# Xinjie-Q/Boosting-NeRV

Hardware: AMD Instinct MI355X
Metric: train frames/sec (higher is better)
Workload: dtype fp32; 1 GPU; NeRV-boost 1.5M (1489577 params, fc_dim 30) train step on a synthetic Bunny-shaped clip 132x3x720x1280: decoder fwd + Fusion10_freq + bwd + fused Adan; frames resident in HBM; global_batch=1, per_gpu_batch=1, parallelism=dp1, hipgraph=True, rccl_ranks=0, collective_in_graph=False

## Files before the change

boosting_nerv_amd/_lib.py:

```python
import ctypes as C
import os

import torch

_HERE = os.path.dirname(os.path.abspath(__file__))
LIB_PATH = os.environ.get("BNERV_LIB") or os.path.join(_HERE, "libbnerv_hip.so")

MAX_DENSE_GROUPS = 40
ADAN_MAX_TENSORS = 48
SFT_CHUNKS = 32
LOSS_STATS = 5
DENSE_DX_CHUNK = 64

ACT_NONE, ACT_RELU, ACT_SIN = 0, 1, 2
IN_PLAIN, IN_AFFINE, IN_GELU_AFFINE, IN_UNSHUFFLE, IN_TANHGRAD = 0, 1, 2, 3, 4
EP_BIAS, EP_BIAS_SIN, EP_BIAS_RES, EP_BIAS_TANH, EP_PLAIN, EP_DGELU, EP_DSIN, EP_BIAS_GELU, EP_DGELU_SAVED = 0, 1, 2, 3, 4, 5, 6, 7, 8
CONV_FAM = ("head1_fwd", "head1_dgrad", "head3", "stem_dgrad", "small", "small96", "wide_bf16", "q4", "generic")
WGRAD_FAM = ("stem", "gemm1x1", "lean", "wide_bf16", "wide_f32", "generic")
PAIR_FORM = ("stem", "q4_lean", "small_wide", "bf16_wide", "head")

_fp = C.c_void_p


class DenseFwdDesc(C.Structure):
# ... 2 lines not shown


class DenseBwdDesc(C.Structure):
    _fields_ = [("x", _fp), ("w", _fp), ("y", _fp), ("aux", _fp), ("dy", _fp), ("dpre", _fp), ("dw", _fp), ("db", _fp),
                ("dx_part", _fp), ("I", C.c_int), ("O", C.c_int), ("act", C.c_int), ("_pad", C.c_int)]


class ConvDesc(C.Structure):
    _fields_ = [("x", _fp), ("w", _fp), ("bias", _fp), ("out", _fp), ("out2", _fp), ("aux0", _fp), ("aux1", _fp),
                ("aux2", _fp), ("scale", _fp), ("shift", _fp), ("partial", _fp),
                ("B", C.c_int), ("Cin", C.c_int), ("Cout", C.c_int), ("H", C.c_int), ("W", C.c_int), ("k", C.c_int),
                ("in_mode", C.c_int), ("ep_mode", C.c_int), ("in_s", C.c_int), ("out_s", C.c_int),
                ("transposed", C.c_int), ("wCo", C.c_int), ("wCi", C.c_int), ("ctx", _fp)]


class TimeBranchMlp(C.Structure):
    _fields_ = [("w1", _fp), ("b1", _fp), ("w2", _fp), ("b2", _fp), ("hs", _fp), ("out", _fp), ("C", C.c_int), ("_pad", C.c_int)]


class TimeBranchDesc(C.Structure):
    _fields_ = [("pos", _fp), ("bases", _fp), ("pe", _fp), ("sw0", _fp), ("sb0", _fp), ("sy0", _fp), ("saux0", _fp),
                ("tw0", _fp), ("tb0", _fp), ("tw1", _fp), ("tb1", _fp), ("ty0", _fp), ("taux0", _fp), ("ty1", _fp), ("taux1", _fp),
                ("B", C.c_int), ("L", C.c_int), ("SH", C.c_int), ("TH", C.c_int), ("TO", C.c_int), ("n_mlp", C.c_int)]


class WgradDesc(C.Structure):
    _fields_ = [("x", _fp), ("g", _fp), ("gaux", _fp), ("scale", _fp), ("shift", _fp), ("dw", _fp), ("db", _fp),
                ("ws", _fp), ("ws_bytes", C.c_size_t),
                ("B", C.c_int), ("Cin", C.c_int), ("Cout", C.c_int), ("H", C.c_int), ("W", C.c_int), ("k", C.c_int),
                ("in_mode", C.c_int), ("g_mode", C.c_int), ("g_s", C.c_int), ("defer_finish", C.c_int), ("ctx", _fp)]


class LossDesc(C.Structure):
    _fields_ = [("pred", _fp), ("target", _fp), ("grad", _fp), ("loss_out", _fp), ("stats_out", _fp), ("ws", _fp),
                ("ws_bytes", C.c_size_t), ("B", C.c_int), ("C", C.c_int), ("H", C.c_int), ("W", C.c_int),
                ("c_l1", C.c_float), ("c_l2", C.c_float), ("c_ms", C.c_float), ("c_fft", C.c_float)]


class AdanChunk(C.Structure):
    _fields_ = [("p", _fp * ADAN_MAX_TENSORS), ("g", _fp * ADAN_MAX_TENSORS), ("exp_avg", _fp * ADAN_MAX_TENSORS),
                ("exp_avg_sq", _fp * ADAN_MAX_TENSORS), ("exp_avg_diff", _fp * ADAN_MAX_TENSORS),
                ("neg_pre_grad", _fp * ADAN_MAX_TENSORS), ("n", C.c_int * ADAN_MAX_TENSORS), ("n_tensors", C.c_int)]


class AdanHyper(C.Structure):
    _fields_ = [("beta1", C.c_float), ("beta2", C.c_float), ("beta3", C.c_float), ("eps", C.c_float),
# ... 106 lines not shown


PRUNE_SLICE = 16384


class PruneItem(C.Structure):
    _fields_ = [("x", _fp), ("mask", _fp), ("n", C.c_uint32), ("_pad", C.c_uint32)]


class YuvCoeffs(C.Structure):
    _fields_ = [("m", C.c_float * 9), ("off", C.c_float * 3), ("scale", C.c_float * 3), ("maxcode", C.c_float)]


_I, _Z, _V, _F = C.c_int, C.c_size_t, C.c_void_p, C.c_float
SYMBOLS = {
    "bnerv_abi_version": (_I, []),
    "bnerv_last_error": (C.c_char_p, []),
    "bnerv_build_arch": (C.c_char_p, []),
    "bnerv_pe_fwd_f32": (_I, [_V, _V, _V, _V, _I, _I]),
    "bnerv_pe_fwd_f64": (_I, [_V, _V, _V, _V, _I, _I]),
    "bnerv_pe_fwd_f32_from_f64": (_I, [_V, _V, _V, _V, _I, _I]),
    "bnerv_dense_grouped_fwd": (_I, [_V, C.POINTER(DenseFwdDesc), _I, _I]),
    "bnerv_time_branch_fwd": (_I, [_V, C.POINTER(TimeBranchDesc), C.POINTER(TimeBranchMlp)]),
    "bnerv_dense_grouped_bwd": (_I, [_V, C.POINTER(DenseBwdDesc), _I, _I]),
    "bnerv_sft_affine_fwd": (_I, [_V, _V, _V, _V, _V, _I, _I, _I]),
    "bnerv_sft_affine_bwd": (_I, [_V, _V, _V, _V, _V, _V, _I, _I, _I]),
    "bnerv_reduce_slabs": (_I, [_V, _V, _I, _I, _V]),
    "bnerv_ctx_create": (_I, [C.POINTER(C.c_void_p)]),
    "bnerv_ctx_destroy": (None, [_V]),
    "bnerv_ctx_scratch_bytes": (_Z, [_V]),
    "bnerv_ctx_reserve": (_I, [_V, _Z]),
    "bnerv_ctx_wplan_record": (_I, [_V]),
    "bnerv_ctx_wplan_freeze": (_I, [_V]),
    "bnerv_ctx_wplan_run": (_I, [_V, _V]),
    "bnerv_ctx_wplan_run_fetch": (_I, [_V, _V, _V, _V, _V, _I, _Z, _V, _V]),
    "bnerv_ctx_wplan_end": (_I, [_V]),
    "bnerv_ctx_wplan_entries": (_I, [_V]),
    "bnerv_reduce_slabs_deferred": (_I, [_V, _V, _V, _I, _I, _V]),
    "bnerv_flush_deferred": (_I, [_V, _V]),
    "bnerv_deferred_pending": (_I, [_V]),
    "bnerv_conv_tiles": (_I, [_I, _I]),
    "bnerv_conv_igemm": (_I, [_V, C.POINTER(ConvDesc)]),
    "bnerv_conv_splitk_ws_bytes": (_Z, [C.POINTER(ConvDesc)]),
    "bnerv_conv_partial_rows": (_I, [C.POINTER(ConvDesc)]),
    "bnerv_conv_family": (_I, [C.POINTER(ConvDesc), C.POINTER(C.c_int)]),
    "bnerv_conv_wgrad_ws_bytes": (_Z, [_I, _I, _I, _I, _I, _I]),
# ... 243 lines not shown
```

boosting_nerv_amd/csrc/abi.hip:

```cpp
#include "common.h"
#include <string.h>

namespace { thread_local char g_err[512] = ""; }

int bnerv_set_error(int code, const char* fmt, ...) {
    va_list ap;
    va_start(ap, fmt);
    vsnprintf(g_err, sizeof(g_err), fmt, ap);
    va_end(ap);
    return code;
}

extern "C" int bnerv_abi_version(void) { return BNERV_ABI_VERSION; }
extern "C" const char* bnerv_last_error(void) { return g_err; }
extern "C" const char* bnerv_build_arch(void) { return "gfx950"; }

#include "sidejob.h"
#include <new>
#include <vector>

namespace {
__global__ __launch_bounds__(256) void side_flush_kernel(const SidePack sp) {
    __shared__ float red[256];
    side_slice<SidePack, true>(sp, blockIdx.x, red);
}
__global__ __launch_bounds__(256) void side_flush_many_kernel(const SideFlushPack sp) {
    __shared__ float red[256];
    side_slice<SideFlushPack, true>(sp, blockIdx.x, red);
}

SideJob make_job(const void* src, int n_slabs, int count, int ncols, float* out, float* out2, const float* fs = nullptr, const float* ft = nullptr) {
    SideJob j;
    j.fs = fs;
    j.ft = ft;
    j.src = reinterpret_cast<const float*>(src);
    j.out = out;
    j.out2 = out2;
    j.n_slabs = n_slabs;
    j.count = count;
    j.ncols = ncols;
    int lanes = 8;
    while (lanes < 128 && lanes * 16 < n_slabs) lanes *= 2;
    j.epb = 256 / lanes;
    j.slices = (count + j.epb - 1) / j.epb;
    return j;
}
}

void bnerv_side_push(bnerv_ctx* ctx, hipStream_t st, const void* src, int n_slabs, int count, int ncols, float* out, float* out2, const float* fold_scale, const float* fold_shift) {
    const SideJob j = make_job(src, n_slabs, count, ncols, out, out2, fold_scale, fold_shift);
    if (ctx) { ctx->queue.push_back(j); return; }
    SidePack sp;
    sp.j[0] = j;
    sp.n_jobs = 1;
    sp.n_slices = j.slices;
    hipLaunchKernelGGL(side_flush_kernel, dim3(sp.n_slices), dim3(256), 0, st, sp);
}

void bnerv_side_take(bnerv_ctx* ctx, SidePack* sp, int max_slices, bool step_over) {
    sp->n_jobs = 0;
    sp->n_slices = 0;
    if (!ctx) return;
    std::vector<SideJob>& q = ctx->queue;
    int n = 0;
    size_t i = 0;
    while (i < q.size() && n < SIDE_MAX_JOBS) {
// ... 86 lines not shown
```

boosting_nerv_amd/csrc/dense.hip:

```cpp
#include "common.h"
#include "sidejob.h"
#include "launch.h"

namespace {

__global__ void pe_f32_kernel(const float* __restrict__ pos, const float* __restrict__ bases, float* __restrict__ out, int N, int L) {
    const int i = blockIdx.x * blockDim.x + threadIdx.x;
    if (i >= N * L) return;
    const int n = i / L, l = i - n * L;
    const float v = __fmul_rn(pos[n], bases[l]);
    out[(size_t)n * 2 * L + l] = sinf(v);
    out[(size_t)n * 2 * L + L + l] = cosf(v);
}
__global__ void pe_f32_from_f64_kernel(const double* __restrict__ pos, const float* __restrict__ bases, float* __restrict__ out, int N, int L) {
    const int i = blockIdx.x * blockDim.x + threadIdx.x;
    if (i >= N * L) return;
    const int n = i / L, l = i - n * L;
    const float v = __fmul_rn((float)pos[n], bases[l]);
    out[(size_t)n * 2 * L + l] = sinf(v);
    out[(size_t)n * 2 * L + L + l] = cosf(v);
}
__global__ void pe_f64_kernel(const double* __restrict__ pos, const float* __restrict__ bases, float* __restrict__ out, int N, int L) {
    const int i = blockIdx.x * blockDim.x + threadIdx.x;
    if (i >= N * L) return;
// ... 16 lines not shown
    for (int b = 0; b < ap->B; ++b) {
        const float* x = g.x + (size_t)b * g.I;
        float s = 0.f;
        for (int i = lane; i < g.I; i += 64) s = fmaf(wrow[i], x[i], s);
        s = wave_sum(s);
        if (lane == 0) {
            const float pre = s + bias;
            float y = pre;
            if (g.act == BNERV_ACT_RELU) y = fmaxf(pre, 0.f);
            else if (g.act == BNERV_ACT_SIN) {
                float sv, cv;
                sincosf(pre, &sv, &cv);
                y = sv;
                if (g.aux) g.aux[(size_t)b * g.O + o] = cv;
            }
            g.y[(size_t)b * g.O + o] = y;
        }
    }
}

struct BwdArgs { bnerv_dense_bwd_desc g[BNERV_MAX_DENSE_GROUPS]; int B; };

constexpr int DW_CHUNK = 1024;
__device__ __forceinline__ void dense_bwd_w_body(const BwdArgs& a, const int bx, const int by, const int bz) {
    const BwdArgs* ap = &a;
    const bnerv_dense_bwd_desc g = a.g[by];
    const int lane = threadIdx.x & 63, wave = threadIdx.x >> 6;
    const int o = bx * 4 + wave;
    const int i0 = bz * DW_CHUNK;
    if (o >= g.O || (i0 >= g.I && bz != 0)) return;
    const int B = ap->B;
    if (bz == 0) {
        float dbsum = 0.f;
        for (int b = 0; b < B; ++b) {
            const size_t k = (size_t)b * g.O + o;
            float dp = g.dy[k];
            if (g.act == BNERV_ACT_RELU) dp = g.y[k] > 0.f ? dp : 0.f;
            else if (g.act == BNERV_ACT_SIN) dp *= g.aux[k];
            if (lane == 0) g.dpre[k] = dp;
            dbsum += dp;
        }
        if (lane == 0 && g.db) g.db[o] = dbsum;
    }
    const int i1 = min(i0 + DW_CHUNK, g.I);
    for (int ib = i0 + lane; ib < i1; ib += 256) {
        float s[4] = {0.f, 0.f, 0.f, 0.f};
        for (int b = 0; b < B; ++b) {
            const size_t k = (size_t)b * g.O + o;
            float dp = g.dy[k];
            if (g.act == BNERV_ACT_RELU) dp = g.y[k] > 0.f ? dp : 0.f;
            else if (g.act == BNERV_ACT_SIN) dp *= g.aux[k];
#pragma unroll
            for (int u = 0; u < 4; ++u) {
                const int i = ib + 64 * u;
                if (i < i1) s[u] = fmaf(dp, g.x[(size_t)b * g.I + i], s[u]);
            }
        }
#pragma unroll
        for (int u = 0; u < 4; ++u) {
            const int i = ib + 64 * u;
            if (i < i1) g.dw[(size_t)o * g.I + i] = s[u];
        }
    }
}

__device__ __forceinline__ void dense_bwd_x_body(const BwdArgs& a, const int bx, const int by, const int bz) {
    const BwdArgs* ap = &a;
    const bnerv_dense_bwd_desc g = a.g[bz];
    if (!g.dx_part) return;
    const int chunk = bx;
    const int o0 = chunk * BNERV_DENSE_DX_CHUNK;
    if (o0 >= g.O) return;
    const int o1 = min(o0 + BNERV_DENSE_DX_CHUNK, g.O);
    const int b = by;
    __shared__ float s_dp[BNERV_DENSE_DX_CHUNK];
    if ((int)threadIdx.x < BNERV_DENSE_DX_CHUNK) {
        float dp = 0.f;
        if ((int)threadIdx.x < o1 - o0) {
            const size_t k = (size_t)b * g.O + o0 + threadIdx.x;
            dp = g.dy[k];
            if (g.act == BNERV_ACT_RELU) dp = g.y[k] > 0.f ? dp : 0.f;
            else if (g.act == BNERV_ACT_SIN) dp *= g.aux[k];
        }
        s_dp[threadIdx.x] = dp;
    }
    __syncthreads();
    for (int i = threadIdx.x; i < g.I; i += 256) {
        float wv[BNERV_DENSE_DX_CHUNK];
#pragma unroll
        for (int r = 0; r < BNERV_DENSE_DX_CHUNK; ++r) wv[r] = o0 + r < o1 ? g.w[(size_t)(o0 + r) * g.I + i] : 0.f;
        float s = 0.f;
#pragma unroll
        for (int r = 0; r < BNERV_DENSE_DX_CHUNK; ++r) s = fmaf(s_dp[r], wv[r], s);
        g.dx_part[((size_t)chunk * ap->B + b) * g.I + i] = s;
    }
}

struct BwdGrid { int nw, wpre[BNERV_MAX_DENSE_GROUPS + 1], xpre[BNERV_MAX_DENSE_GROUPS + 1]; int n_groups, B; };
__global__ __launch_bounds__(256) void dense_bwd_kernel(const BwdArgs a, const BwdGrid q) {
    int t = blockIdx.x;
    const int* pre = t < q.nw ? q.wpre : q.xpre;
    const bool wphase = t < q.nw;
    if (!wphase) t -= q.nw;
    const int ln = threadIdx.x & 63;
    const bool ge = ln + 1 < q.n_groups && t >= pre[ln + 1];
// ... 226 lines not shown
        s_t0[b][r] = sv;
        if (cb == 0) { d.ty0[(size_t)b * d.TH + r] = sv; d.taux0[(size_t)b * d.TH + r] = cv; }
    }
    __syncthreads();
    tb_rows16<TB_MAXT>(w_t1, b_t1, d.TH, TO, s_t0, &s_zt[0][0], TB_MAXT, B);
    __syncthreads();
    for (int e = tid; e < B * TO; e += TB_NT) {
        const int b = e / TO, r = e - b * TO;
        float sv, cv;
        sincosf(s_zt[b][r], &sv, &cv);
        s_zt[b][r] = sv;
        if (cb == 0) { d.ty1[(size_t)b * TO + r] = sv; d.taux1[(size_t)b * TO + r] = cv; }
    }
    __syncthreads();
    tb_multi8(nm, TO, TO, B, [&](int) { return TO; }, [&](int k) { return w_m + k * mstride; }, [&](int k) { return b_m + k * bstride; },
              [&](int, int b) { return &s_zt[b][0]; },
              [&](int k, int r, int b, float v) { const float y = fmaxf(v, 0.f); s_h[k][b][r] = y; a.m[m0 + k].hs[(size_t)b * TO + r] = y; });
    __syncthreads();
    tb_multi8(nm, a.cmax, TO, B, [&](int k) { return a.m[m0 + k].C; }, [&](int k) { return w_m + k * mstride + TO * TO; }, [&](int k) { return b_m + k * bstride + TB_MAXO; },
              [&](int k, int b) { return &s_h[k][b][0]; },
              [&](int k, int r, int b, float v) { a.m[m0 + k].out[(size_t)b * a.m[m0 + k].C + r] = v; });
}

extern "C" int bnerv_dense_grouped_fwd(void* stream, const bnerv_dense_fwd_desc* groups, int n_groups, int B) {
    BNERV_REQUIRE(groups && n_groups > 0 && n_groups <= BNERV_MAX_DENSE_GROUPS && B > 0, "dense_grouped_fwd: bad args (n_groups=%d)", n_groups);
    FwdArgs a;
    a.B = B;
    int maxO = 0;
    for (int i = 0; i < n_groups; ++i) {
        BNERV_REQUIRE(groups[i].x && groups[i].w && groups[i].y && groups[i].I > 0 && groups[i].O > 0, "dense_grouped_fwd: bad group %d", i);
        a.g[i] = groups[i];
        if (groups[i].O > maxO) maxO = groups[i].O;
    }
    hipStream_t st = (hipStream_t)stream;
    hipLaunchKernelGGL(dense_fwd_kernel, dim3(cdiv(maxO, 4), n_groups), dim3(256), 0, st, a);
    BNERV_LAUNCH_CHECK("dense_fwd");
    return BNERV_OK;
}

extern "C" int bnerv_dense_grouped_bwd(void* stream, const bnerv_dense_bwd_desc* groups, int n_groups, int B) {
    BNERV_REQUIRE(groups && n_groups > 0 && n_groups <= BNERV_MAX_DENSE_GROUPS && B > 0 && B <= 65535, "dense_grouped_bwd: bad args (n_groups=%d)", n_groups);
    BwdArgs a;
    a.B = B;
    int maxO = 0, maxI = 0;
    bool any_dx = false;
    for (int i = 0; i < n_groups; ++i) {
// ... 56 lines not shown
    if (d.B > TB_MAXB || 2 * d.L > TB_MAXI || d.SH > 4096 || d.TH > TB_MAXT || d.TO > TB_MAXO || d.n_mlp > BNERV_MAX_DENSE_GROUPS) return 1;
    if ((2 * d.L) % 4 || d.TH % 4 || d.TO % 4 || !aligned16(d.tw0, d.tw1)) return 1;
    TBArgs a;
    a.d = d;
    a.cmax = 4;
    for (int i = 0; i < d.n_mlp; ++i) {
        BNERV_REQUIRE(mlps[i].w1 && mlps[i].w2 && mlps[i].hs && mlps[i].out && mlps[i].C > 0, "time_branch_fwd: bad modulation MLP %d", i);
        if (((mlps[i].C + 3) & ~3) > a.cmax) a.cmax = (mlps[i].C + 3) & ~3;
        if (mlps[i].C > TB_MAXC || !aligned16(mlps[i].w1, mlps[i].w2)) return 1;
        a.m[i].w1 = mlps[i].w1; a.m[i].b1 = mlps[i].b1; a.m[i].w2 = mlps[i].w2; a.m[i].b2 = mlps[i].b2; a.m[i].hs = mlps[i].hs; a.m[i].out = mlps[i].out;
        a.m[i].C = mlps[i].C; a.m[i]._pad = 0;
    }
    a.rows_per_block = 16;
    a.nb_stem = cdiv(d.SH, a.rows_per_block);
    a.mlps_per_block = d.n_mlp > 32 ? TB_MAXM : 2;
    a.nb_chain = d.n_mlp > 0 ? cdiv(d.n_mlp, a.mlps_per_block) : 1;
    const size_t lds = ((size_t)d.TH * 2 * d.L + (size_t)d.TO * d.TH + (size_t)a.mlps_per_block * ((size_t)d.TO * d.TO + (size_t)a.cmax * d.TO)) * sizeof(float);
    if (lds > 100 * 1024) return 1;
    if (const int rc = dyn_lds<&time_branch_kernel>(lds, "time_branch")) return rc;
    hipLaunchKernelGGL(time_branch_kernel, dim3(a.nb_stem + a.nb_chain), dim3(TB_NT), lds, (hipStream_t)stream, a);
    BNERV_LAUNCH_CHECK("time_branch");
    return BNERV_OK;
}
```

boosting_nerv_amd/csrc/sidejob.h:

```cpp
#pragma once
#include "common.h"

constexpr int SIDE_MAX_JOBS = 4;

struct SideJob {
    const float* src;
    float* out;
    float* out2;
    int n_slabs, count, ncols;
    int epb;
    int slices;
    const float* fs;
    const float* ft;
};

struct SidePack {
    SideJob j[SIDE_MAX_JOBS];
    int n_jobs, n_slices;
};
constexpr int SIDE_FLUSH_JOBS = 32;
struct SideFlushPack {
    SideJob j[SIDE_FLUSH_JOBS];
    int n_jobs, n_slices;
    int start[SIDE_FLUSH_JOBS];
};

#include <vector>
struct bnerv_ctx {
    std::vector<SideJob> queue;
    void* scratch = nullptr;
    size_t scratch_bytes = 0;
    struct BfWPlan* wplan = nullptr;
};
void bnerv_wplan_free(bnerv_ctx* ctx);
void* bnerv_ctx_scratch(bnerv_ctx* ctx, size_t bytes, hipStream_t st);

void bnerv_side_push(bnerv_ctx* ctx, hipStream_t st, const void* src, int n_slabs, int count, int ncols, float* out, float* out2,
                     const float* fold_scale = nullptr, const float* fold_shift = nullptr);
void bnerv_side_take(bnerv_ctx* ctx, SidePack* sp, int max_slices, bool step_over = false);
int bnerv_side_flush(bnerv_ctx* ctx, hipStream_t st);
int bnerv_side_pending(const bnerv_ctx* ctx);

// ... 90 lines not shown
```

boosting_nerv_amd/ops.py:

```python
import ctypes as C
import os

import torch
import torch.nn.functional as F

from . import _lib as L


def _ws(nbytes, device):
    return torch.empty(max(int(nbytes), 16), dtype=torch.uint8, device=device)


_STREAM_CTX = object()
_SUMS_EP = (L.EP_DGELU, L.EP_DSIN, L.EP_DGELU_SAVED)


def _conv_desc(x, w, bias, out, *, B, Cin, Cout, H, W, k, in_mode, ep_mode, in_s=1, out_s=1, transposed=0, out2=None,
               aux0=None, aux1=None, aux2=None, scale=None, shift=None, partial=None, ctx=_STREAM_CTX):
    return L.ConvDesc(L.ptr(x), L.ptr(w), L.ptr(bias), L.ptr(out), L.ptr(out2), L.ptr(aux0), L.ptr(aux1), L.ptr(aux2),
                      L.ptr(scale), L.ptr(shift), L.ptr(partial), B, Cin, Cout, H, W, k, in_mode, ep_mode, in_s, out_s,
                      transposed, w.shape[0], w.shape[1], L.ctx().handle if ctx is _STREAM_CTX else ctx)


def _wgrad_desc(x, g, dw, db, ws, ws_bytes, *, B, Cin, Cout, H, W, k, in_mode, g_mode, g_s=1, gaux=None, scale=None, shift=None,
# ... 267 lines not shown

    @staticmethod
    def backward(ctx, dy):
        _enter_backward(reads_sums=True)
        x2, w2, y, aux = ctx.saved_tensors
        B, I = x2.shape
        O = w2.shape[0]
        dy = L.f32c(dy).reshape(B, O)
        dw = torch.empty(O, I, dtype=torch.float32, device=x2.device)
        db = torch.empty(O, dtype=torch.float32, device=x2.device) if ctx.has_b else None
        dx = torch.empty(B, I, dtype=torch.float32, device=x2.device) if ctx.needs_input_grad[0] else None
        lib = L.load()
        nbytes = lib.bnerv_dense_gemm_bwd_ws_bytes(B, I, O)
        ws = _ws(nbytes, x2.device) if nbytes else None
        L.check(lib.bnerv_dense_gemm_bwd(L.stream(), L.ptr(x2), L.ptr(w2), L.ptr(y), L.ptr(aux), L.ptr(dy), L.ptr(dx), L.ptr(dw), L.ptr(db),
                                         L.ptr(ws), nbytes, B, I, O, ctx.act), "bnerv_dense_gemm_bwd")
        return (None if dx is None else dx.reshape(ctx.xshape)), dw.reshape(ctx.wshape), db, None


def dense_gemm(x, w, b, act="none"):
    return _DenseGemm.apply(x, w, b, _ACT[act])


class _TimeBranch(torch.autograd.Function):

    @staticmethod
    def forward(ctx, pos, bases, n_mlp, *params):
        lib = L.load()
        dev = pos.device
        B, Lv = pos.shape[0], bases.numel()
        p2 = [L.f32c(t).reshape(t.shape[0], -1) if t.dim() > 1 else L.f32c(t) for t in params]
        sw0, sb0, sw1, sb1, tw0, tb0, tw1, tb1 = p2[:8]
        mw = p2[8:]
        SH, SO, TH, TO = sw0.shape[0], sw1.shape[0], tw0.shape[0], tw1.shape[0]
        f = lambda *sh: torch.empty(*sh, dtype=torch.float32, device=dev)
        pe, sy0, saux0, sy1, saux1 = f(B, 2 * Lv), f(B, SH), f(B, SH), f(B, SO), f(B, SO)
        ty0, taux0, ty1, taux1 = f(B, TH), f(B, TH), f(B, TO), f(B, TO)
        hs = [f(B, TO) for _ in range(n_mlp)]
        outs = [f(B, mw[4 * i + 2].shape[0]) for i in range(n_mlp)]
        d = L.TimeBranchDesc(L.ptr(pos), L.ptr(bases), L.ptr(pe), L.ptr(sw0), L.ptr(sb0), L.ptr(sy0), L.ptr(saux0),
                             L.ptr(tw0), L.ptr(tb0), L.ptr(tw1), L.ptr(tb1), L.ptr(ty0), L.ptr(taux0), L.ptr(ty1), L.ptr(taux1), B, Lv, SH, TH, TO, n_mlp)
        ml = (L.TimeBranchMlp * max(n_mlp, 1))()
        for i in range(n_mlp):
            w1, b1, w2, b2 = mw[4 * i:4 * i + 4]
            ml[i].w1, ml[i].b1, ml[i].w2, ml[i].b2 = w1.data_ptr(), b1.data_ptr(), w2.data_ptr(), b2.data_ptr()
            ml[i].hs, ml[i].out, ml[i].C = hs[i].data_ptr(), outs[i].data_ptr(), w2.shape[0]
# ... 2 lines not shown
            L.check(rc if rc < 0 else -1, "bnerv_time_branch_fwd (shapes were checked by ops.time_branch)")
        g = (L.DenseFwdDesc * 1)(L.DenseFwdDesc(L.ptr(sy0), L.ptr(sw1), L.ptr(sb1), L.ptr(sy1), L.ptr(saux1), SH, SO, L.ACT_SIN, 0))
        L.check(lib.bnerv_dense_grouped_fwd(L.stream(), g, 1, B), "bnerv_dense_grouped_fwd")
        ctx.n_mlp, ctx.B = n_mlp, B
        ctx.pshapes = [tuple(t.shape) for t in params]
        ctx.save_for_backward(pe, sy0, saux0, sy1, saux1, ty0, taux0, ty1, taux1, *hs, *outs, *p2)
        ctx.set_materialize_grads(False)
        return (sy1, ty1, *outs)

    @staticmethod
    def backward(ctx, d_sy1, d_ty1, *d_outs):
        _enter_backward(reads_sums=True)
        n, B = ctx.n_mlp, ctx.B
        sv = ctx.saved_tensors
        pe, sy0, saux0, sy1, saux1, ty0, taux0, ty1, taux1 = sv[:9]
        hs, outs, p2 = sv[9:9 + n], sv[9 + n:9 + 2 * n], sv[9 + 2 * n:]
        sw0, sb0, sw1, sb1, tw0, tb0, tw1, tb1 = p2[:8]
        mw = p2[8:]
        none, relu, sin = L.ACT_NONE, L.ACT_RELU, L.ACT_SIN
        g = [None] * len(p2)
        w1s, w2s = [mw[4 * i] for i in range(n)], [mw[4 * i + 2] for i in range(n)]
        if n + 1 > L.MAX_DENSE_GROUPS or n == 0:
            raise L.BnervError("time branch backward: group count outside the grouped kernel's table")
        dxa, dwa, dba = _dense_grouped_bwd([none] * n + [sin], list(hs) + [sy0], w2s + [sw1], list(outs) + [sy1], [None] * n + [saux1],
                                           list(d_outs) + [d_sy1], [True] * (n + 1), [True] * (n + 1), False, B, defer_reduce=True)
        dx4, d_sy0 = dxa[:n], dxa[n]
        if any(w.shape[0] > L.DENSE_DX_CHUNK for w in w2s):
            _flush_deferred()
        dx3, dw3, db3 = _dense_grouped_bwd([relu] * n, [ty1] * n, w1s, hs, [None] * n, dx4, [True] * n, [True] * n, True, B, defer_reduce=True)
        _flush_deferred()
        tot = next(t for t in dx3 if t is not None)
        d_zt = tot if d_ty1 is None else tot + L.f32c(d_ty1).reshape(tot.shape)
        for i in range(n):
            g[8 + 4 * i], g[8 + 4 * i + 1], g[8 + 4 * i + 2], g[8 + 4 * i + 3] = dw3[i], db3[i], dwa[i], dba[i]
        dxb, dwb, dbb = _dense_grouped_bwd([sin, sin], [ty0, pe], [tw1, sw0], [ty1, sy0], [taux1, saux0], [d_zt, d_sy0], [True, False], [True, True], False, B)
        _, dwc, dbc = _dense_grouped_bwd([sin], [pe], [tw0], [ty0], [taux0], [dxb[0]], [False], [True], False, B)
        g[0], g[1], g[2], g[3] = dwb[1], dbb[1], dwa[n], dba[n]
        g[4], g[5], g[6], g[7] = dwc[0], dbc[0], dwb[0], dbb[0]
        g = [None if t is None else t.reshape(sh) for t, sh in zip(g, ctx.pshapes)]
        return (None, None, None, *g)


def time_branch(pos, bases, stem, stem_t, mlps):
    if os.environ.get("BNERV_TIME_BRANCH", "1") == "0" or pos.dtype != torch.float64 or not pos.is_cuda or pos.dim() != 1:
        return None
    B, Lv = pos.shape[0], bases.numel()
# ... 1714 lines not shown
```

include/bnerv.h:

```cpp
#ifndef BNERV_H
#define BNERV_H

#include <stddef.h>
#include <stdint.h>

#ifdef __cplusplus
extern "C" {
#endif

#define BNERV_ABI_VERSION 9

#define BNERV_OK 0
#define BNERV_E_ARG (-1)
#define BNERV_E_LAUNCH (-2)
#define BNERV_E_WS (-3)

int bnerv_abi_version(void);
const char* bnerv_last_error(void);
const char* bnerv_build_arch(void);

int bnerv_pe_fwd_f32(void* stream, const float* pos, const float* bases, float* out, int N, int L);
int bnerv_pe_fwd_f64(void* stream, const double* pos, const float* bases, float* out, int N, int L);
int bnerv_pe_fwd_f32_from_f64(void* stream, const double* pos, const float* bases, float* out, int N, int L);

// ... 21 lines not shown
    float* dw;
    float* db;
    float* dx_part;
    int I, O, act, _pad;
} bnerv_dense_bwd_desc;

#define BNERV_DENSE_DX_CHUNK 64

int bnerv_dense_grouped_fwd(void* stream, const bnerv_dense_fwd_desc* groups, int n_groups, int B);
int bnerv_dense_grouped_bwd(void* stream, const bnerv_dense_bwd_desc* groups, int n_groups, int B);

typedef struct { const float* w1; const float* b1; const float* w2; const float* b2; float* hs; float* out; int C; int _pad; } bnerv_time_branch_mlp;
typedef struct {
    const double* pos;
    const float* bases;
    float* pe;
    const float* sw0; const float* sb0;
    float* sy0; float* saux0;
    const float* tw0; const float* tb0; const float* tw1; const float* tb1;
    float* ty0; float* taux0; float* ty1; float* taux1;
    int B, L, SH, TH, TO, n_mlp;
} bnerv_time_branch_desc;
int bnerv_time_branch_fwd(void* stream, const bnerv_time_branch_desc* d, const bnerv_time_branch_mlp* mlps );

#define BNERV_SFT_CHUNKS 32
int bnerv_sft_affine_fwd(void* stream, const float* x, const float* scale, const float* shift, float* y, int B, int C, int HW);
int bnerv_sft_affine_bwd(void* stream, const float* x, const float* scale, const float* g, float* dx, float* part, int B, int C, int HW);

int bnerv_lncf_fwd(void* stream, const float* x, const float* w, const float* b, float* y, int B, int C, int HW, float eps);
size_t bnerv_lncf_bwd_ws_bytes(int B, int C, int HW);
int bnerv_lncf_bwd(void* stream, const float* x, const float* w, const float* dy, float* dx, float* dwb, void* ws, size_t ws_bytes,
                   int B, int C, int HW, float eps);

int bnerv_reduce_slabs(void* stream, const float* slabs, int n_slabs, int count, float* out);

typedef struct bnerv_ctx bnerv_ctx;
int bnerv_ctx_create(bnerv_ctx** out);
void bnerv_ctx_destroy(bnerv_ctx* ctx);
size_t bnerv_ctx_scratch_bytes(const bnerv_ctx* ctx);
int bnerv_ctx_reserve(bnerv_ctx* ctx, size_t bytes);
int bnerv_ctx_wplan_record(bnerv_ctx* ctx);
int bnerv_ctx_wplan_freeze(bnerv_ctx* ctx);
int bnerv_ctx_wplan_run(bnerv_ctx* ctx, void* stream);
int bnerv_ctx_wplan_run_fetch(bnerv_ctx* ctx, void* stream, const float* clip, const double* norms, const float* sel_dev, int n_frames, size_t frame_elems,
                              float* dst_img, double* dst_norm);
int bnerv_ctx_wplan_end(bnerv_ctx* ctx);
// ... 346 lines not shown
```

Measured before the change: 696.7 frames/s.

## Fuse time-branch backward into two launches covering modulation MLPs and stem

Replaces the chain of grouped dense backward calls, deferred slab reductions and flushes for the time-embedding branch with two dedicated kernels. The first computes each modulation MLP's backward in one block and runs the stem layer's dx/dw bodies in the same grid. The second reduces the partial slabs and finishes the stem and temporal MLP weight and bias gradients. This cuts kernel launches and intermediate host-side orchestration on a tiny, latency-bound part of the step, at the cost of more specialised code with shape limits and a fallback path.

```diff
diff --git a/boosting_nerv_amd/_lib.py b/boosting_nerv_amd/_lib.py
--- a/boosting_nerv_amd/_lib.py
+++ b/boosting_nerv_amd/_lib.py
@@ -48,6 +48,22 @@
     _fields_ = [("pos", _fp), ("bases", _fp), ("pe", _fp), ("sw0", _fp), ("sb0", _fp), ("sy0", _fp), ("saux0", _fp),
                 ("tw0", _fp), ("tb0", _fp), ("tw1", _fp), ("tb1", _fp), ("ty0", _fp), ("taux0", _fp), ("ty1", _fp), ("taux1", _fp),
                 ("B", C.c_int), ("L", C.c_int), ("SH", C.c_int), ("TH", C.c_int), ("TO", C.c_int), ("n_mlp", C.c_int)]
+
+
+class TimeBranchBwdMlp(C.Structure):
+    _fields_ = [("w1", _fp), ("w2", _fp), ("hs", _fp), ("d_out", _fp), ("dw1", _fp), ("db1", _fp), ("dw2", _fp), ("db2", _fp),
+                ("C", C.c_int), ("_pad", C.c_int)]
+
+
+class TimeBranchBwdDesc(C.Structure):
+    _fields_ = [("pe", _fp), ("sw1", _fp), ("sy0", _fp), ("saux0", _fp), ("saux1", _fp), ("d_sy1", _fp),
+                ("tw1", _fp), ("ty0", _fp), ("taux0", _fp), ("ty1", _fp), ("taux1", _fp), ("d_ty1", _fp),
+                ("d_sw0", _fp), ("d_sb0", _fp), ("d_sw1", _fp), ("d_sb1", _fp), ("d_tw0", _fp), ("d_tb0", _fp), ("d_tw1", _fp), ("d_tb1", _fp),
+                ("sx_part", _fp), ("zt_part", _fp), ("s_dpre", _fp),
+                ("B", C.c_int), ("L", C.c_int), ("SH", C.c_int), ("SO", C.c_int), ("TH", C.c_int), ("TO", C.c_int), ("n_mlp", C.c_int), ("_pad", C.c_int)]
+
+
+TIME_BRANCH_BWD_MLP_BYTES, TIME_BRANCH_BWD_DESC_BYTES = 72, 216
 
 
 class WgradDesc(C.Structure):
@@ -200,6 +216,7 @@
     "bnerv_pe_fwd_f32_from_f64": (_I, [_V, _V, _V, _V, _I, _I]),
     "bnerv_dense_grouped_fwd": (_I, [_V, C.POINTER(DenseFwdDesc), _I, _I]),
     "bnerv_time_branch_fwd": (_I, [_V, C.POINTER(TimeBranchDesc), C.POINTER(TimeBranchMlp)]),
+    "bnerv_time_branch_bwd": (_I, [_V, C.POINTER(TimeBranchBwdDesc), C.POINTER(TimeBranchBwdMlp)]),
     "bnerv_dense_grouped_bwd": (_I, [_V, C.POINTER(DenseBwdDesc), _I, _I]),
     "bnerv_sft_affine_fwd": (_I, [_V, _V, _V, _V, _V, _I, _I, _I]),
     "bnerv_sft_affine_bwd": (_I, [_V, _V, _V, _V, _V, _V, _I, _I, _I]),
diff --git a/boosting_nerv_amd/csrc/abi.hip b/boosting_nerv_amd/csrc/abi.hip
--- a/boosting_nerv_amd/csrc/abi.hip
+++ b/boosting_nerv_amd/csrc/abi.hip
@@ -39,9 +39,7 @@
     j.n_slabs = n_slabs;
     j.count = count;
     j.ncols = ncols;
-    int lanes = 8;
-    while (lanes < 128 && lanes * 16 < n_slabs) lanes *= 2;
-    j.epb = 256 / lanes;
+    j.epb = side_epb(n_slabs);
     j.slices = (count + j.epb - 1) / j.epb;
     return j;
 }
diff --git a/boosting_nerv_amd/csrc/dense.hip b/boosting_nerv_amd/csrc/dense.hip
--- a/boosting_nerv_amd/csrc/dense.hip
+++ b/boosting_nerv_amd/csrc/dense.hip
@@ -62,8 +62,9 @@
 struct BwdArgs { bnerv_dense_bwd_desc g[BNERV_MAX_DENSE_GROUPS]; int B; };
 
 constexpr int DW_CHUNK = 1024;
-__device__ __forceinline__ void dense_bwd_w_body(const BwdArgs& a, const int bx, const int by, const int bz) {
-    const BwdArgs* ap = &a;
+template <class Args>
+__device__ __forceinline__ void dense_bwd_w_body(const Args& a, const int bx, const int by, const int bz) {
+    const Args* ap = &a;
     const bnerv_dense_bwd_desc g = a.g[by];
     const int lane = threadIdx.x & 63, wave = threadIdx.x >> 6;
     const int o = bx * 4 + wave;
@@ -76,7 +77,7 @@
             const size_t k = (size_t)b * g.O + o;
             float dp = g.dy[k];
             if (g.act == BNERV_ACT_RELU) dp = g.y[k] > 0.f ? dp : 0.f;
-            else if (g.act == BNERV_ACT_SIN) dp *= g.aux[k];
+            else if (g.act == BNERV_ACT_SIN) dp = __fmul_rn(dp, g.aux[k]);
             if (lane == 0) g.dpre[k] = dp;
             dbsum += dp;
         }
@@ -89,7 +90,7 @@
             const size_t k = (size_t)b * g.O + o;
             float dp = g.dy[k];
             if (g.act == BNERV_ACT_RELU) dp = g.y[k] > 0.f ? dp : 0.f;
-            else if (g.act == BNERV_ACT_SIN) dp *= g.aux[k];
+            else if (g.act == BNERV_ACT_SIN) dp = __fmul_rn(dp, g.aux[k]);
 #pragma unroll
             for (int u = 0; u < 4; ++u) {
                 const int i = ib + 64 * u;
@@ -104,8 +105,9 @@
     }
 }
 
-__device__ __forceinline__ void dense_bwd_x_body(const BwdArgs& a, const int bx, const int by, const int bz) {
-    const BwdArgs* ap = &a;
+template <class Args>
+__device__ __forceinline__ void dense_bwd_x_body(const Args& a, const int bx, const int by, const int bz) {
+    const Args* ap = &a;
     const bnerv_dense_bwd_desc g = a.g[bz];
     if (!g.dx_part) return;
     const int chunk = bx;
@@ -120,7 +122,7 @@
             const size_t k = (size_t)b * g.O + o0 + threadIdx.x;
             dp = g.dy[k];
             if (g.act == BNERV_ACT_RELU) dp = g.y[k] > 0.f ? dp : 0.f;
-            else if (g.act == BNERV_ACT_SIN) dp *= g.aux[k];
+            else if (g.act == BNERV_ACT_SIN) dp = __fmul_rn(dp, g.aux[k]);
         }
         s_dp[threadIdx.x] = dp;
     }
@@ -393,6 +395,244 @@
               [&](int k, int r, int b, float v) { a.m[m0 + k].out[(size_t)b * a.m[m0 + k].C + r] = v; });
 }
 
+struct Bwd1Args { bnerv_dense_bwd_desc g[1]; int B; };
+struct TBBMlp { const float* w1; const float* w2; const float* hs; const float* dout; float* dw1; float* db1; float* dw2; float* db2; int C; int _pad; };
+constexpr int TBB_MAX_MLP = BNERV_MAX_DENSE_GROUPS - 1;
+struct TBBArgsA {
+    Bwd1Args stem;
+    TBBMlp m[TBB_MAX_MLP];
+    const float* zt;
+    float* zt_part;
+    int nw, wx, nx, xx;
+    int n_mlp, TO;
+};
+struct TBBArgsB {
+    const float* pe; const float* saux0; const float* sx_part;
+    const float* zt_part; const float* d_ty1; const float* taux1; const float* ty0; const float* tw1; const float* taux0;
+    float* d_sw0; float* d_sb0; float* d_tw1; float* d_tb1; float* d_tw0; float* d_tb0;
+    int B, I, SH, TH, TO, n_sx, n_mlp, nb_stem, epb_sx, epb_zt;
+};
+static_assert(sizeof(TBBMlp) == BNERV_TIME_BRANCH_BWD_MLP_BYTES && sizeof(bnerv_time_branch_bwd_mlp) == BNERV_TIME_BRANCH_BWD_MLP_BYTES, "time branch backward: MLP entry");
+static_assert(sizeof(bnerv_time_branch_bwd_desc) == BNERV_TIME_BRANCH_BWD_DESC_BYTES, "time branch backward: descriptor");
+static_assert(sizeof(TBBArgsA) <= 4096 && sizeof(TBBArgsB) <= 4096, "time branch backward: kernel-argument segment");
+constexpr int TBB_NT = 256, TBB_ROWS = 32;
+
+__device__ __forceinline__ float tbb_pad_rows(const float s, const int nr) { return nr < BNERV_DENSE_DX_CHUNK ? s + 0.f : s; }
+
+__device__ __forceinline__ void tbb_mod_block(const TBBArgsA& a, const int mi) {
+    __shared__ float s_w2[TB_MAXC * TB_MAXO], s_w1[TB_MAXO * TB_MAXO];
+    __shared__ float s_dp2[TB_MAXB][TB_MAXC], s_hs[TB_MAXB][TB_MAXO], s_zt[TB_MAXB][TB_MAXO], s_dp1[TB_MAXB][TB_MAXO];
+    __shared__ float s_xp[TB_MAXC / BNERV_DENSE_DX_CHUNK][TB_MAXB][TB_MAXO];
+    const TBBMlp m = a.m[mi];
+    const int tid = threadIdx.x, B = a.stem.B, TO = a.TO, C = m.C;
+    constexpr int NW2 = TB_MAXC * TB_MAXO / TBB_NT, NW1 = TB_MAXO * TB_MAXO / TBB_NT, NDP = TB_MAXB * TB_MAXC / TBB_NT;
+    float r_w2[NW2], r_w1[NW1], r_dp[NDP];
+#pragma unroll
+    for (int u = 0; u < NW2; ++u) r_w2[u] = tid + u * TBB_NT < C * TO ? m.w2[tid + u * TBB_NT] : 0.f;
+#pragma unroll
+    for (int u = 0; u < NW1; ++u) r_w1[u] = tid + u * TBB_NT < TO * TO ? m.w1[tid + u * TBB_NT] : 0.f;
+#pragma unroll
+    for (int u = 0; u < NDP; ++u) r_dp[u] = m.dout && tid + u * TBB_NT < B * C ? m.dout[tid + u * TBB_NT] : 0.f;
+    const float r_hs = tid < B * TO ? m.hs[tid] : 0.f, r_zt = tid < B * TO ? a.zt[tid] : 0.f;
+#pragma unroll
+    for (int u = 0; u < NW2; ++u) s_w2[tid + u * TBB_NT] = r_w2[u];
+#pragma unroll
+    for (int u = 0; u < NW1; ++u) s_w1[tid + u * TBB_NT] = r_w1[u];
+#pragma unroll
+    for (int u = 0; u < NDP; ++u)
+        if (tid + u * TBB_NT < B * C) s_dp2[(tid + u * TBB_NT) / C][(tid + u * TBB_NT) % C] = r_dp[u];
+    if (tid < B * TO) { s_hs[tid / TO][tid % TO] = r_hs; s_zt[tid / TO][tid % TO] = r_zt; }
+    __syncthreads();
+    for (int o = tid; o < C; o += TBB_NT) {
+        float s = 0.f;
+        for (int b = 0; b < B; ++b) s += s_dp2[b][o];
+        m.db2[o] = s;
+    }
+    for (int e = tid; e < C * TO; e += TBB_NT) {
+        const int o = e / TO, i = e - o * TO;
+        float s = 0.f;
+        for (int b = 0; b < B; ++b) s = fmaf(s_dp2[b][o], s_hs[b][i], s);
+        m.dw2[e] = s;
+    }
+    const int nch = (C + BNERV_DENSE_DX_CHUNK - 1) / BNERV_DENSE_DX_CHUNK;
+    for (int e = tid; e < nch * B * TO; e += TBB_NT) {
+        const int ch = e / (B * TO), b = (e - ch * B * TO) / TO, i = e % TO;
+        const int o0 = ch * BNERV_DENSE_DX_CHUNK, nr = min(BNERV_DENSE_DX_CHUNK, C - o0);
+        float s = 0.f;
+#pragma unroll 8
+        for (int r = 0; r < nr; ++r) s = fmaf(s_dp2[b][o0 + r], s_w2[(o0 + r) * TO + i], s);
+        s_xp[ch][b][i] = tbb_pad_rows(s, nr);
+    }
+    __syncthreads();
+    for (int e = tid; e < B * TO; e += TBB_NT) {
+        const int b = e / TO, r = e - b * TO;
+        const float dh = nch == 1 ? s_xp[0][b][r] : (0.f + s_xp[0][b][r]) + s_xp[1][b][r];
+        s_dp1[b][r] = s_hs[b][r] > 0.f ? dh : 0.f;
+    }
+    __syncthreads();
+    for (int r = tid; r < TO; r += TBB_NT) {
+        float s = 0.f;
+        for (int b = 0; b < B; ++b) s += s_dp1[b][r];
+        m.db1[r] = s;
+    }
+    for (int e = tid; e < TO * TO; e += TBB_NT) {
+        const int r = e / TO, i = e - r * TO;
+        float s = 0.f;
+        for (int b = 0; b < B; ++b) s = fmaf(s_dp1[b][r], s_zt[b][i], s);
+        m.dw1[e] = s;
+    }
+    for (int e = tid; e < B * TO; e += TBB_NT) {
+        const int b = e / TO, i = e - b * TO;
+        float s = 0.f;
+#pragma unroll 8
+        for (int r = 0; r < TO; ++r) s = fmaf(s_dp1[b][r], s_w1[r * TO + i], s);
+        a.zt_part[((size_t)mi * B + b) * TO + i] = tbb_pad_rows(s, TO);
+    }
+}
+
+__global__ __launch_bounds__(TBB_NT) void time_branch_bwd_a_kernel(const TBBArgsA a) {
+    int t = blockIdx.x;
+    if (t < a.n_mlp) { tbb_mod_block(a, t); return; }
+    t -= a.n_mlp;
+    if (t < a.nx) { dense_bwd_x_body(a.stem, t % a.xx, t / a.xx, 0); return; }
+    t -= a.nx;
+    if (t < a.nw) dense_bwd_w_body(a.stem, t % a.wx, 0, t / a.wx);
+}
+
+__device__ __forceinline__ float tbb_slab_lane_sum(const float* __restrict__ src, const int n_slabs, const size_t count, const size_t i, const bool live,
+                                                   const int epb) {
+    const int lanes = TBB_NT / epb, lane = threadIdx.x / epb;
+    float acc = 0.f;
+    if (live) {
+        const float* p = src + i;
+        for (int k0 = lane; k0 < n_slabs; k0 += 16 * lanes) {
+            float v[16];
+#pragma unroll
+            for (int u = 0; u < 16; ++u) {
+                const int k = k0 + u * lanes;
+                v[u] = k < n_slabs ? p[(size_t)k * count] : 0.f;
+            }
+#pragma unroll
+            for (int w = 8; w >= 1; w >>= 1)
+#pragma unroll
+                for (int u = 0; u < w; ++u) v[u] += v[u + w];
+            acc += v[0];
+        }
+    }
+    return acc;
+}
+__device__ __forceinline__ float tbb_slab_combine(const float acc, const bool live, const int epb, float* red) {
+    const int lanes = TBB_NT / epb, e = threadIdx.x % epb, lane = threadIdx.x / epb;
+    red[lane * epb + e] = acc;
+    __syncthreads();
+    float t = 0.f;
+    if (lane == 0 && live)
+        for (int l = 0; l < lanes; ++l) t += red[l * epb + e];
+    __syncthreads();
+    return t;
+}
+
+__global__ __launch_bounds__(TBB_NT) void time_branch_bwd_b_kernel(const TBBArgsB a) {
+    __shared__ float red[TBB_NT];
+    __shared__ float s_pe[TB_MAXB * TB_MAXI];
+    __shared__ float s_d[TB_MAXB][TB_MAXT];
+    __shared__ float s_d0[TB_MAXB][TB_MAXT];
+    __shared__ float s_ty0[TB_MAXB * TB_MAXT], s_a0[TB_MAXB * TB_MAXT], s_a1[TB_MAXB * TB_MAXO], s_dt[TB_MAXB * TB_MAXO];
+    __shared__ float s_tw1[TB_MAXO * TB_MAXT];
+    const int tid = threadIdx.x, B = a.B, I = a.I, TO = a.TO, TH = a.TH;
+    float r_pe[TB_MAXB * TB_MAXI / TBB_NT];
+#pragma unroll
+    for (int u = 0; u < TB_MAXB * TB_MAXI / TBB_NT; ++u) r_pe[u] = tid + u * TBB_NT < B * I ? a.pe[tid + u * TBB_NT] : 0.f;
+    if ((int)blockIdx.x < a.nb_stem) {
+        const int o0 = (int)blockIdx.x * TBB_ROWS, epb = a.epb_sx;
+        const int e = tid % epb, lane = tid / epb;
+        for (int p0 = 0; p0 < B * TBB_ROWS; p0 += epb) {
+            const int idx = p0 + e, b = idx / TBB_ROWS, r = idx - b * TBB_ROWS, o = o0 + r;
+            const bool live = o < a.SH;
+            const size_t k = (size_t)b * a.SH + (live ? o : 0);
+            const float aux = lane == 0 && live ? a.saux0[k] : 0.f;
+            const float acc = tbb_slab_lane_sum(a.sx_part, a.n_sx, (size_t)B * a.SH, k, live, epb);
+            if (p0 == 0) {
+#pragma unroll
+                for (int u = 0; u < TB_MAXB * TB_MAXI / TBB_NT; ++u) s_pe[tid + u * TBB_NT] = r_pe[u];
+            }
+            const float t = tbb_slab_combine(acc, live, epb, red);
+            if (lane == 0 && live) s_d[b][r] = __fmul_rn(t, aux);
+        }
+        __syncthreads();
+        for (int r = tid; r < TBB_ROWS && o0 + r < a.SH; r += TBB_NT) {
+            float s = 0.f;
+            for (int b = 0; b < B; ++b) s += s_d[b][r];
+            a.d_sb0[o0 + r] = s;
+        }
+        for (int e2 = tid; e2 < TBB_ROWS * I; e2 += TBB_NT) {
+            const int r = e2 / I, i = e2 - r * I;
+            if (o0 + r >= a.SH) break;
+            float s = 0.f;
+            for (int b = 0; b < B; ++b) s = fmaf(s_d[b][r], s_pe[b * I + i], s);
+            a.d_sw0[(size_t)(o0 + r) * I + i] = s;
+        }
+        return;
+    }
+    {
+        float r_w[TB_MAXO * TB_MAXT / TBB_NT];
+#pragma unroll
+        for (int u = 0; u < TB_MAXO * TB_MAXT / TBB_NT; ++u) r_w[u] = tid + u * TBB_NT < TO * TH ? a.tw1[tid + u * TBB_NT] : 0.f;
+        const float r_y0 = tid < B * TH ? a.ty0[tid] : 0.f, r_a0 = tid < B * TH ? a.taux0[tid] : 0.f;
+        const float r_a1 = tid < B * TO ? a.taux1[tid] : 0.f, r_dt = a.d_ty1 && tid < B * TO ? a.d_ty1[tid] : 0.f;
+        const int epb = a.epb_zt, e = tid % epb, lane = tid / epb;
+        for (int p0 = 0; p0 < B * TO; p0 += epb) {
+            const int idx = p0 + e;
+            const bool live = idx < B * TO;
+            const float acc = tbb_slab_lane_sum(a.zt_part, a.n_mlp, (size_t)B * TO, live ? idx : 0, live, epb);
+            if (p0 == 0) {
+#pragma unroll
+                for (int u = 0; u < TB_MAXB * TB_MAXI / TBB_NT; ++u) s_pe[tid + u * TBB_NT] = r_pe[u];
+#pragma unroll
+                for (int u = 0; u < TB_MAXO * TB_MAXT / TBB_NT; ++u) s_tw1[tid + u * TBB_NT] = r_w[u];
+                s_ty0[tid] = r_y0; s_a0[tid] = r_a0;
+                if (tid < TB_MAXB * TB_MAXO) { s_a1[tid] = r_a1; s_dt[tid] = r_dt; }
+            }
+            const float t = tbb_slab_combine(acc, live, epb, red);
+            if (lane == 0 && live) {
+                const float dz = a.d_ty1 ? t + s_dt[idx] : t;
+                s_d[idx / TO][idx % TO] = __fmul_rn(dz, s_a1[idx]);
+            }
+        }
+    }
+    __syncthreads();
+    for (int r = tid; r < TO; r += TBB_NT) {
+        float s = 0.f;
+        for (int b = 0; b < B; ++b) s += s_d[b][r];
+        a.d_tb1[r] = s;
+    }
+    for (int e = tid; e < TO * TH; e += TBB_NT) {
+        const int r = e / TH, i = e - r * TH;
+        float s = 0.f;
+        for (int b = 0; b < B; ++b) s = fmaf(s_d[b][r], s_ty0[b * TH + i], s);
+        a.d_tw1[e] = s;
+    }
+    for (int e = tid; e < B * TH; e += TBB_NT) {
+        const int b = e / TH, i = e - b * TH;
+        float s = 0.f;
+#pragma unroll 8
+        for (int r = 0; r < TO; ++r) s = fmaf(s_d[b][r], s_tw1[r * TH + i], s);
+        s_d0[b][i] = __fmul_rn(tbb_pad_rows(s, TO), s_a0[e]);
+    }
+    __syncthreads();
+    for (int r = tid; r < TH; r += TBB_NT) {
+        float s = 0.f;
+        for (int b = 0; b < B; ++b) s += s_d0[b][r];
+        a.d_tb0[r] = s;
+    }
+    for (int e = tid; e < TH * I; e += TBB_NT) {
+        const int r = e / I, i = e - r * I;
+        float s = 0.f;
+        for (int b = 0; b < B; ++b) s = fmaf(s_d0[b][r], s_pe[b * I + i], s);
+        a.d_tw0[e] = s;
+    }
+}
+
 extern "C" int bnerv_dense_grouped_fwd(void* stream, const bnerv_dense_fwd_desc* groups, int n_groups, int B) {
     BNERV_REQUIRE(groups && n_groups > 0 && n_groups <= BNERV_MAX_DENSE_GROUPS && B > 0, "dense_grouped_fwd: bad args (n_groups=%d)", n_groups);
     FwdArgs a;
@@ -495,3 +735,42 @@
     BNERV_LAUNCH_CHECK("time_branch");
     return BNERV_OK;
 }
+
+extern "C" int bnerv_time_branch_bwd(void* stream, const bnerv_time_branch_bwd_desc* dp, const bnerv_time_branch_bwd_mlp* mlps) {
+    BNERV_REQUIRE(dp && mlps, "time_branch_bwd: null descriptor");
+    const bnerv_time_branch_bwd_desc& d = *dp;
+    BNERV_REQUIRE(d.n_mlp > 0, "time_branch_bwd: needs at least one modulation MLP (n_mlp=%d)", d.n_mlp);
+    BNERV_REQUIRE(d.pe && d.sw1 && d.sy0 && d.saux0 && d.saux1 && d.d_sy1 && d.tw1 && d.ty0 && d.taux0 && d.ty1 && d.taux1, "time_branch_bwd: null tensor");
+    BNERV_REQUIRE(d.d_sw0 && d.d_sb0 && d.d_sw1 && d.d_sb1 && d.d_tw0 && d.d_tb0 && d.d_tw1 && d.d_tb1, "time_branch_bwd: null gradient output");
+    BNERV_REQUIRE(d.sx_part && d.zt_part && d.s_dpre, "time_branch_bwd: null scratch");
+    BNERV_REQUIRE(d.B > 0 && d.L > 0 && d.SH > 0 && d.SO > 0 && d.TH > 0 && d.TO > 0, "time_branch_bwd: bad shape");
+    if (d.B > TB_MAXB || 2 * d.L > TB_MAXI || d.SH > 4096 || d.TH > TB_MAXT || d.TO > TB_MAXO || d.n_mlp > TBB_MAX_MLP) return 1;
+    TBBArgsA a{};
+    for (int i = 0; i < d.n_mlp; ++i) {
+        const bnerv_time_branch_bwd_mlp& m = mlps[i];
+        BNERV_REQUIRE(m.w1 && m.w2 && m.hs && m.dw1 && m.db1 && m.dw2 && m.db2 && m.C > 0, "time_branch_bwd: bad modulation MLP %d", i);
+        if (m.C > TB_MAXC) return 1;
+        a.m[i].w1 = m.w1; a.m[i].w2 = m.w2; a.m[i].hs = m.hs; a.m[i].dout = m.d_out;
+        a.m[i].dw1 = m.dw1; a.m[i].db1 = m.db1; a.m[i].dw2 = m.dw2; a.m[i].db2 = m.db2; a.m[i].C = m.C; a.m[i]._pad = 0;
+    }
+    bnerv_dense_bwd_desc& g = a.stem.g[0];
+    g.x = d.sy0; g.w = d.sw1; g.y = nullptr; g.aux = d.saux1; g.dy = d.d_sy1; g.dpre = d.s_dpre; g.dw = d.d_sw1; g.db = d.d_sb1; g.dx_part = d.sx_part;
+    g.I = d.SH; g.O = d.SO; g.act = BNERV_ACT_SIN; g._pad = 0;
+    a.stem.B = d.B;
+    a.zt = d.ty1; a.zt_part = d.zt_part;
+    a.wx = cdiv(d.SO, 4); a.nw = a.wx * cdiv(d.SH, DW_CHUNK);
+    a.xx = cdiv(d.SO, BNERV_DENSE_DX_CHUNK); a.nx = a.xx * d.B;
+    a.n_mlp = d.n_mlp; a.TO = d.TO;
+    TBBArgsB b;
+    b.pe = d.pe; b.saux0 = d.saux0; b.sx_part = d.sx_part; b.zt_part = d.zt_part; b.d_ty1 = d.d_ty1; b.taux1 = d.taux1; b.ty0 = d.ty0; b.tw1 = d.tw1;
+    b.taux0 = d.taux0; b.d_sw0 = d.d_sw0; b.d_sb0 = d.d_sb0; b.d_tw1 = d.d_tw1; b.d_tb1 = d.d_tb1; b.d_tw0 = d.d_tw0; b.d_tb0 = d.d_tb0;
+    b.B = d.B; b.I = 2 * d.L; b.SH = d.SH; b.TH = d.TH; b.TO = d.TO; b.n_sx = a.xx; b.n_mlp = d.n_mlp;
+    b.nb_stem = cdiv(d.SH, TBB_ROWS);
+    b.epb_sx = side_epb(b.n_sx); b.epb_zt = side_epb(b.n_mlp);
+    hipStream_t st = (hipStream_t)stream;
+    hipLaunchKernelGGL(time_branch_bwd_a_kernel, dim3(a.nw + a.nx + a.n_mlp), dim3(TBB_NT), 0, st, a);
+    BNERV_LAUNCH_CHECK("time_branch_bwd_a");
+    hipLaunchKernelGGL(time_branch_bwd_b_kernel, dim3(b.nb_stem + 1), dim3(TBB_NT), 0, st, b);
+    BNERV_LAUNCH_CHECK("time_branch_bwd_b");
+    return BNERV_OK;
+}
diff --git a/boosting_nerv_amd/csrc/sidejob.h b/boosting_nerv_amd/csrc/sidejob.h
--- a/boosting_nerv_amd/csrc/sidejob.h
+++ b/boosting_nerv_amd/csrc/sidejob.h
@@ -18,6 +18,11 @@
     SideJob j[SIDE_MAX_JOBS];
     int n_jobs, n_slices;
 };
+static inline int side_epb(int n_slabs) {
+    int lanes = 8;
+    while (lanes < 128 && lanes * 16 < n_slabs) lanes *= 2;
+    return 256 / lanes;
+}
 constexpr int SIDE_FLUSH_JOBS = 32;
 struct SideFlushPack {
     SideJob j[SIDE_FLUSH_JOBS];
diff --git a/boosting_nerv_amd/ops.py b/boosting_nerv_amd/ops.py
--- a/boosting_nerv_amd/ops.py
+++ b/boosting_nerv_amd/ops.py
@@ -313,6 +313,40 @@
     return _DenseGemm.apply(x, w, b, _ACT[act])
 
 
+TIME_BRANCH_BWD_CALLS = {"taken": 0, "declined": 0}
+
+
+def _time_branch_bwd_two_launches(B, saved, hs, p2, d_sy1, d_ty1, d_outs):
+    pe, sy0, saux0, sy1, saux1, ty0, taux0, ty1, taux1 = saved
+    sw0, sb0, sw1, sb1, tw0, tb0, tw1, tb1 = p2[:8]
+    mw = p2[8:]
+    n = len(hs)
+    dev = pe.device
+    SH, SO, TH, TO = sw0.shape[0], sw1.shape[0], tw0.shape[0], tw1.shape[0]
+    f = lambda *sh: torch.empty(*sh, dtype=torch.float32, device=dev)
+    g = [f(*t.shape) for t in p2]
+    nch = (SO + L.DENSE_DX_CHUNK - 1) // L.DENSE_DX_CHUNK
+    sx_part, zt_part, s_dpre = f(nch, B, SH), f(n, B, TO), f(B, SO)
+    d_sy1 = L.f32c(d_sy1).reshape(B, SO)
+    d_ty1 = None if d_ty1 is None else L.f32c(d_ty1).reshape(B, TO)
+    douts = [None if t is None else L.f32c(t).reshape(B, -1) for t in d_outs]
+    d = L.TimeBranchBwdDesc(L.ptr(pe), L.ptr(sw1), L.ptr(sy0), L.ptr(saux0), L.ptr(saux1), L.ptr(d_sy1),
+                            L.ptr(tw1), L.ptr(ty0), L.ptr(taux0), L.ptr(ty1), L.ptr(taux1), L.ptr(d_ty1),
+                            L.ptr(g[0]), L.ptr(g[1]), L.ptr(g[2]), L.ptr(g[3]), L.ptr(g[4]), L.ptr(g[5]), L.ptr(g[6]), L.ptr(g[7]),
+                            L.ptr(sx_part), L.ptr(zt_part), L.ptr(s_dpre), B, pe.shape[1] // 2, SH, SO, TH, TO, n, 0)
+    ml = (L.TimeBranchBwdMlp * n)()
+    for i in range(n):
+        w1, _, w2, _ = mw[4 * i:4 * i + 4]
+        dw1, db1, dw2, db2 = g[8 + 4 * i:12 + 4 * i]
+        ml[i].w1, ml[i].w2, ml[i].hs, ml[i].d_out = w1.data_ptr(), w2.data_ptr(), hs[i].data_ptr(), L.ptr(douts[i])
+        ml[i].dw1, ml[i].db1, ml[i].dw2, ml[i].db2, ml[i].C = dw1.data_ptr(), db1.data_ptr(), dw2.data_ptr(), db2.data_ptr(), w2.shape[0]
+    rc = L.load().bnerv_time_branch_bwd(L.stream(), C.byref(d), ml)
+    if rc == 1:
+        return None
+    L.check(rc, "bnerv_time_branch_bwd")
+    return g
+
+
 class _TimeBranch(torch.autograd.Function):
 
     @staticmethod
@@ -361,6 +395,11 @@
         w1s, w2s = [mw[4 * i] for i in range(n)], [mw[4 * i + 2] for i in range(n)]
         if n + 1 > L.MAX_DENSE_GROUPS or n == 0:
             raise L.BnervError("time branch backward: group count outside the grouped kernel's table")
+        if os.environ.get("BNERV_TIME_BRANCH_BWD", "1") != "0":
+            g2 = _time_branch_bwd_two_launches(B, sv[:9], hs, p2, d_sy1, d_ty1, d_outs)
+            TIME_BRANCH_BWD_CALLS["taken" if g2 is not None else "declined"] += 1
+            if g2 is not None:
+                return (None, None, None, *[t.reshape(sh) for t, sh in zip(g2, ctx.pshapes)])
         dxa, dwa, dba = _dense_grouped_bwd([none] * n + [sin], list(hs) + [sy0], w2s + [sw1], list(outs) + [sy1], [None] * n + [saux1],
                                            list(d_outs) + [d_sy1], [True] * (n + 1), [True] * (n + 1), False, B, defer_reduce=True)
         dx4, d_sy0 = dxa[:n], dxa[n]
diff --git a/include/bnerv.h b/include/bnerv.h
--- a/include/bnerv.h
+++ b/include/bnerv.h
@@ -67,6 +67,28 @@
     int B, L, SH, TH, TO, n_mlp;
 } bnerv_time_branch_desc;
 int bnerv_time_branch_fwd(void* stream, const bnerv_time_branch_desc* d, const bnerv_time_branch_mlp* mlps );
+
+#define BNERV_TIME_BRANCH_BWD_MLP_BYTES 72
+#define BNERV_TIME_BRANCH_BWD_DESC_BYTES 216
+typedef struct {
+    const float* w1; const float* w2;
+    const float* hs;
+    const float* d_out;
+    float* dw1; float* db1; float* dw2; float* db2;
+    int C; int _pad;
+} bnerv_time_branch_bwd_mlp;
+typedef struct {
+    const float* pe;
+    const float* sw1; const float* sy0; const float* saux0; const float* saux1;
+    const float* d_sy1;
+    const float* tw1; const float* ty0; const float* taux0; const float* ty1; const float* taux1;
+    const float* d_ty1;
+    float* d_sw0; float* d_sb0; float* d_sw1; float* d_sb1;
+    float* d_tw0; float* d_tb0; float* d_tw1; float* d_tb1;
+    float* sx_part; float* zt_part; float* s_dpre;
+    int B, L, SH, SO, TH, TO, n_mlp, _pad;
+} bnerv_time_branch_bwd_desc;
+int bnerv_time_branch_bwd(void* stream, const bnerv_time_branch_bwd_desc* d, const bnerv_time_branch_bwd_mlp* mlps );
 
 #define BNERV_SFT_CHUNKS 32
 int bnerv_sft_affine_fwd(void* stream, const float* x, const float* scale, const float* shift, float* y, int B, int C, int HW);
```

Measured after the change: 704.3 frames/s (median of 6 runs). +1.1%, better.
